# Nostrademous/dotaclient

Measured on AMD Instinct MI355X. Metric: PPO optimizer samples/sec (whole node) + actor steps/sec, 1v1-mid LSTM policy, higher is better.
Workload: dtype fp32

## Files before the change

dotaclient_amd/ops/csrc/dx_chain.hip:

```cpp
#include "common.h"
#include <cstdlib>

namespace {

using dca::bf16x8;
using dca::f32x4;

constexpr int BM = 48, BK = 32, NT = 512, P = 256, XC = 128, RD = 4;
constexpr int NI1 = BM / 16;

template <bool EXACT>
struct Lay {
  static constexpr int RP = EXACT ? 144 : 64;
  static constexpr int IMG = EXACT ? 1 : 2;
  static constexpr int A1 = BM * RP;
  static constexpr int B1 = P * RP;
  static constexpr int S1 = IMG * (A1 + B1);
  static constexpr int D = IMG * (P / BK) * A1;
  static constexpr int B2 = XC * RP;
  static constexpr int S2 = IMG * B2;
  static constexpr int BYTES = (2 * S1 > D + 2 * S2) ? 2 * S1 : D + 2 * S2;
};

template <bool EXACT>
__device__ __forceinline__ int coff(int r, int c) {
  if constexpr (EXACT) return r * Lay<true>::RP + 16 * c;
  else return r * 64 + 16 * (c ^ ((r >> 1) & 3));
}

__device__ __forceinline__ __amdgpu_buffer_rsrc_t rsrc(const void* p, long long bytes) {
  const unsigned long long a = (unsigned long long)p;
  const unsigned lo = __builtin_amdgcn_readfirstlane((unsigned)a);
  const unsigned hi = __builtin_amdgcn_readfirstlane((unsigned)(a >> 32));
  const int nb = (int)(bytes > 0x7fff0000LL ? 0x7fff0000LL : bytes);
  return __builtin_amdgcn_make_buffer_rsrc((void*)(((unsigned long long)hi << 32) | lo), (short)0,
                                           __builtin_amdgcn_readfirstlane(nb), 0x00020000);
}
__device__ __forceinline__ uint4 ld16(__amdgpu_buffer_rsrc_t r, int off) {
  return __builtin_bit_cast(uint4, __builtin_amdgcn_raw_buffer_load_b128(r, off, 0, 0));
}
constexpr int kOob = 0x7fff8000;

__device__ __forceinline__ unsigned pack2(short a, short b) {
  return (unsigned)(unsigned short)a | ((unsigned)(unsigned short)b << 16);
}
__device__ __forceinline__ void split4(const float4 v, uint2& hi, uint2& lo) {
  const short h0 = dca::f2bf(v.x), h1 = dca::f2bf(v.y), h2 = dca::f2bf(v.z), h3 = dca::f2bf(v.w);
  hi = make_uint2(pack2(h0, h1), pack2(h2, h3));
  lo = make_uint2(pack2(dca::f2bf(v.x - dca::bf2f(h0)), dca::f2bf(v.y - dca::bf2f(h1))),
                  pack2(dca::f2bf(v.z - dca::bf2f(h2)), dca::f2bf(v.w - dca::bf2f(h3))));
}

struct Frag {
  bf16x8 hi, lo;
  float f[8];
};
template <bool EXACT>
__device__ __forceinline__ void get_frag(const char* img, int img_bytes, int r, int q, Frag& fr) {
  if constexpr (EXACT) {
    const float4 a = *reinterpret_cast<const float4*>(img + coff<true>(r, 2 * q));
    const float4 b = *reinterpret_cast<const float4*>(img + coff<true>(r, 2 * q + 1));
    fr.f[0] = a.x; fr.f[1] = a.y; fr.f[2] = a.z; fr.f[3] = a.w;
    fr.f[4] = b.x; fr.f[5] = b.y; fr.f[6] = b.z; fr.f[7] = b.w;
  } else {
    const int o = coff<false>(r, q);
    fr.hi = *reinterpret_cast<const bf16x8*>(img + o);
    fr.lo = *reinterpret_cast<const bf16x8*>(img + img_bytes + o);
  }
}
template <bool EXACT, int NI, int NJ>
__device__ __forceinline__ void mma_tiles(const Frag (&fa)[NI], const Frag (&fb)[NJ], f32x4 (&acc)[NI][NJ]) {
  if constexpr (EXACT) {
#pragma unroll
    for (int e = 0; e < 8; ++e)
#pragma unroll
      for (int i = 0; i < NI; ++i)
#pragma unroll
        for (int j = 0; j < NJ; ++j)
          acc[i][j] = __builtin_amdgcn_mfma_f32_16x16x4f32(fa[i].f[e], fb[j].f[e], acc[i][j], 0, 0, 0);
  } else {
#pragma unroll
    for (int i = 0; i < NI; ++i)
#pragma unroll
      for (int j = 0; j < NJ; ++j) acc[i][j] = __builtin_amdgcn_mfma_f32_16x16x32_bf16(fa[i].lo, fb[j].hi, acc[i][j], 0, 0, 0);
#pragma unroll
    for (int i = 0; i < NI; ++i)
#pragma unroll
      for (int j = 0; j < NJ; ++j) acc[i][j] = __builtin_amdgcn_mfma_f32_16x16x32_bf16(fa[i].hi, fb[j].lo, acc[i][j], 0, 0, 0);
#pragma unroll
    for (int i = 0; i < NI; ++i)
#pragma unroll
      for (int j = 0; j < NJ; ++j) acc[i][j] = __builtin_amdgcn_mfma_f32_16x16x32_bf16(fa[i].hi, fb[j].hi, acc[i][j], 0, 0, 0);
  }
}

template <bool EXACT, int EPI>
__global__ __launch_bounds__(NT, 1) void dpre_dx_kernel(const float* __restrict__ dG, const void* __restrict__ w1h,
                                                        const void* __restrict__ w1l, const float* __restrict__ x,
                                                        const void* __restrict__ w2h, const void* __restrict__ w2l,
                                                        float* __restrict__ dpre, float* __restrict__ dx, int N,
                                                        int K1, int X) {
  using L = Lay<EXACT>;
  constexpr int ES = EXACT ? 4 : 2;
  __shared__ __attribute__((aligned(16))) char lds[L::BYTES];
  const int tid = threadIdx.x, w = tid >> 6, lane = tid & 63, r16 = lane & 15, q = lane >> 4;
  const int r0 = blockIdx.x * BM;
  const __amdgpu_buffer_rsrc_t rA = rsrc(dG, (long long)N * K1 * 4);
  const __amdgpu_buffer_rsrc_t rW1h = rsrc(w1h, (long long)P * K1 * ES);
  const __amdgpu_buffer_rsrc_t rW1l = rsrc(EXACT ? w1h : w1l, (long long)P * K1 * ES);
  const __amdgpu_buffer_rsrc_t rW2h = rsrc(w2h, (long long)X * P * ES);
  const __amdgpu_buffer_rsrc_t rW2l = rsrc(EXACT ? w2h : w2l, (long long)X * P * ES);

  char* dimg = lds;
  constexpr int DIMG = (P / BK) * L::A1;
  if (K1 > 0) {
  const int ar = tid >> 3, ak = (tid & 7) * 4;
  const int arow = r0 + ar;
  const int a_off0 = (ar < BM && arow < N) ? (arow * K1 + ak) * 4 : kOob;
  const int br = tid & 255, bh = tid >> 8;
  const int b_off0 = (br * K1 + 16 * bh) * ES;
  float4 sa[RD];
  uint4 sb[RD][4];
  auto load1 = [&](int slot, int k0) {
    const bool in = k0 < K1;
    sa[slot] = __builtin_bit_cast(float4, ld16(rA, (in && a_off0 != kOob) ? a_off0 + k0 * 4 : kOob));
    if constexpr (EXACT) {
#pragma unroll
      for (int i = 0; i < 4; ++i) sb[slot][i] = ld16(rW1h, in ? b_off0 + (k0 + 4 * i) * 4 : kOob);
    } else {
      const int o = (k0 / BK) * (P * 64) + tid * 16;
#pragma unroll
      for (int j = 0; j < 2; ++j) {
        sb[slot][j] = ld16(rW1h, in ? o + 8192 * j : kOob);
        sb[slot][2 + j] = ld16(rW1l, in ? o + 8192 * j : kOob);
      }
    }
  };
  auto store1 = [&](int slot, int buf) {
    char* base = lds + buf * L::S1;
    char* bb = base + L::IMG * L::A1;
    if constexpr (EXACT) {
      if (ar < BM) *reinterpret_cast<float4*>(base + ar * L::RP + ak * 4) = sa[slot];
#pragma unroll
      for (int i = 0; i < 4; ++i) *reinterpret_cast<uint4*>(bb + br * L::RP + (16 * bh + 4 * i) * 4) = sb[slot][i];
    } else {
      uint2 hi, lo;
      split4(sa[slot], hi, lo);
      const int o = coff<false>(ar, ak >> 3) + 8 * ((ak >> 2) & 1);
      if (ar < BM) {
        *reinterpret_cast<uint2*>(base + o) = hi;
        *reinterpret_cast<uint2*>(base + L::A1 + o) = lo;
      }
#pragma unroll
      for (int j = 0; j < 2; ++j) {
        const int ob = coff<false>(128 * j + (tid >> 2), tid & 3);
        *reinterpret_cast<uint4*>(bb + ob) = sb[slot][j];
        *reinterpret_cast<uint4*>(bb + L::B1 + ob) = sb[slot][2 + j];
      }
    }
  };
  const int wc = w;
  f32x4 acc[NI1][2];
#pragma unroll
  for (int i = 0; i < NI1; ++i)
#pragma unroll
    for (int j = 0; j < 2; ++j) acc[i][j] = f32x4{0.f, 0.f, 0.f, 0.f};
  const int nk = K1 / BK;
#pragma unroll
  for (int d = 0; d < RD; ++d) load1(d, d * BK);
  store1(0, 0);
  __syncthreads();
  for (int ks0 = 0; ks0 < nk; ks0 += RD) {
#pragma unroll
    for (int d = 0; d < RD; ++d) {
      const int ks = ks0 + d;
      const char* base = lds + (d & 1) * L::S1;
      const char* bb = base + L::IMG * L::A1;
      Frag fa[NI1], fb[2];
#pragma unroll
      for (int i = 0; i < NI1; ++i) get_frag<EXACT>(base, L::A1, i * 16 + r16, q, fa[i]);
#pragma unroll
      for (int j = 0; j < 2; ++j) get_frag<EXACT>(bb, L::B1, wc * 32 + j * 16 + r16, q, fb[j]);
      mma_tiles<EXACT, NI1, 2>(fa, fb, acc);
      store1((d + 1) % RD, (d + 1) & 1);
      load1(d, (ks + RD) * BK);
      __syncthreads();
    }
  }

  {
    const __amdgpu_buffer_rsrc_t rX = rsrc(x, EPI == 0 ? (long long)N * P * 4 : (long long)P * 4);
    float xv[NI1][2][4];
#pragma unroll
    for (int i = 0; i < NI1; ++i)
#pragma unroll
      for (int j = 0; j < 2; ++j)
#pragma unroll
        for (int e = 0; e < 4; ++e) {
          const int row = i * 16 + 4 * q + e, col = wc * 32 + j * 16 + r16;
          const int grow = r0 + row;
          if constexpr (EPI == 0) {
            xv[i][j][e] = __builtin_bit_cast(float, __builtin_amdgcn_raw_buffer_load_b32(
                              rX, grow < N ? (grow * P + col) * 4 : kOob, 0, 0));
          } else {
            xv[i][j][e] = e == 0 && i == 0 ? __builtin_bit_cast(float, __builtin_amdgcn_raw_buffer_load_b32(
                                                                           rX, col * 4, 0, 0))
                                           : 0.f;
          }
        }
    const __amdgpu_buffer_rsrc_t rD = rsrc(dpre, (long long)N * P * 4);
#pragma unroll
    for (int i = 0; i < NI1; ++i)
#pragma unroll
      for (int j = 0; j < 2; ++j)
#pragma unroll
        for (int e = 0; e < 4; ++e) {
          const int row = i * 16 + 4 * q + e, col = wc * 32 + j * 16 + r16;
          const int grow = r0 + row;
          float v;
          if constexpr (EPI == 0) v = xv[i][j][e] > 0.f ? acc[i][j][e] : 0.f;
          else if constexpr (EPI == 1) v = fmaxf(acc[i][j][e] + xv[0][j][0], 0.f);
          else v = acc[i][j][e] + xv[0][j][0];
          if (grow >= N) v = 0.f;
          __builtin_amdgcn_raw_buffer_store_b32(__builtin_bit_cast(unsigned, v), rD,
                                                grow < N ? (grow * P + col) * 4 : kOob, 0, 0);
          const int kk = col & (BK - 1);
          char* slab = dimg + (col / BK) * L::A1;
          if constexpr (EXACT) {
            *reinterpret_cast<float*>(slab + coff<true>(row, kk >> 2) + 4 * (kk & 3)) = v;
          } else {
            const int o = coff<false>(row, kk >> 3) + 2 * (kk & 7);
            const short h = dca::f2bf(v);
            *reinterpret_cast<short*>(slab + o) = h;
            *reinterpret_cast<short*>(slab + DIMG + o) = dca::f2bf(v - dca::bf2f(h));
          }
        }
  }

  } else if constexpr (EXACT) {
    for (int i = tid; i < BM * P / 4; i += NT) {
      const int row = i / (P / 4), c4 = (i % (P / 4)) * 4;
      const int grow = r0 + row;
      const float4 v = grow < N ? *reinterpret_cast<const float4*>(dG + (size_t)grow * P + c4)
                                : make_float4(0.f, 0.f, 0.f, 0.f);
      const int kk = c4 & (BK - 1);
      *reinterpret_cast<float4*>(dimg + (c4 / BK) * L::A1 + coff<true>(row, kk >> 2)) = v;
    }
  } else {
    for (int i = tid; i < BM * P / 4; i += NT) {
      const int row = i / (P / 4), c4 = (i % (P / 4)) * 4;
      const int grow = r0 + row;
      const float4 v = grow < N ? *reinterpret_cast<const float4*>(dG + (size_t)grow * P + c4)
                                : make_float4(0.f, 0.f, 0.f, 0.f);
      uint2 hi, lo;
      split4(v, hi, lo);
      const int kk = c4 & (BK - 1);
      char* slab = dimg + (c4 / BK) * L::A1;
      const int o = coff<false>(row, kk >> 3) + 2 * (kk & 7);
      *reinterpret_cast<uint2*>(slab + o) = hi;
      *reinterpret_cast<uint2*>(slab + DIMG + o) = lo;
    }
  }

  if (X == 0) return;
  char* s2 = lds + L::D;
  constexpr int nk2 = P / BK;
  const int nchunk = X / XC, total = nchunk * nk2;
  const int cr = tid & 127, cq = tid >> 7;
  uint4 sw[RD][2];
  auto load2 = [&](int slot, int it) {
    const int c0 = (it / nk2) * XC, kb = it % nk2;
    if constexpr (EXACT) {
      const int o = it < total ? ((c0 + cr) * P + kb * BK + 8 * cq) * ES : kOob;
      sw[slot][0] = ld16(rW2h, o);
      sw[slot][1] = ld16(rW2h, o + 16);
    } else {
      const int o = it < total ? (kb * X + c0) * 64 + tid * 16 : kOob;
      sw[slot][0] = ld16(rW2h, o);
      sw[slot][1] = ld16(rW2l, o);
    }
  };
  auto store2 = [&](int slot, int buf) {
    char* bb = s2 + buf * L::S2;
    if constexpr (EXACT) {
      *reinterpret_cast<uint4*>(bb + coff<true>(cr, 2 * cq)) = sw[slot][0];
      *reinterpret_cast<uint4*>(bb + coff<true>(cr, 2 * cq + 1)) = sw[slot][1];
    } else {
      const int o = coff<false>(tid >> 2, tid & 3);
      *reinterpret_cast<uint4*>(bb + o) = sw[slot][0];
      *reinterpret_cast<uint4*>(bb + L::B2 + o) = sw[slot][1];
    }
  };
  const int vc = w;
  f32x4 acc2[NI1][1];
#pragma unroll
  for (int i = 0; i < NI1; ++i) acc2[i][0] = f32x4{0.f, 0.f, 0.f, 0.f};
  const __amdgpu_buffer_rsrc_t rDx = rsrc(dx, (long long)N * X * 4);
#pragma unroll
  for (int d = 0; d < RD; ++d) load2(d, d);
  store2(0, 0);
  __syncthreads();
  for (int it0 = 0; it0 < total; it0 += RD) {
#pragma unroll
    for (int d = 0; d < RD; ++d) {
      const int it = it0 + d;
      const int chunk = it / nk2, ks = it % nk2;
      const char* bb = s2 + (d & 1) * L::S2;
      Frag fa[NI1], fb[1];
#pragma unroll
      for (int i = 0; i < NI1; ++i) get_frag<EXACT>(dimg + ks * L::A1, DIMG, i * 16 + r16, q, fa[i]);
      get_frag<EXACT>(bb, L::B2, vc * 16 + r16, q, fb[0]);
      mma_tiles<EXACT, NI1, 1>(fa, fb, acc2);
      store2((d + 1) % RD, (d + 1) & 1);
      load2(d, it + RD);
      if (ks == nk2 - 1) {
#pragma unroll
        for (int i = 0; i < NI1; ++i) {
#pragma unroll
          for (int e = 0; e < 4; ++e) {
            const int grow = r0 + i * 16 + 4 * q + e;
            const float v = acc2[i][0][e];
            __builtin_amdgcn_raw_buffer_store_b32(__builtin_bit_cast(unsigned, v), rDx,
                                                  grow < N ? (grow * X + chunk * XC + vc * 16 + r16) * 4 : kOob, 0, 0);
          }
          acc2[i][0] = f32x4{0.f, 0.f, 0.f, 0.f};
        }
      }
      __syncthreads();
    }
  }
}

__global__ __launch_bounds__(256) void split_bf16x2_kernel(const float4* __restrict__ src, uint2* __restrict__ hi,
                                                           uint2* __restrict__ lo, int n4) {
  const int i = blockIdx.x * 256 + threadIdx.x;
  if (i < n4) split4(src[i], hi[i], lo[i]);
}

__global__ __launch_bounds__(256) void split_bf16x2_blk_kernel(const float4* __restrict__ src, uint2* __restrict__ hi,
                                                               uint2* __restrict__ lo, int R, int K) {
  const int i = blockIdx.x * 256 + threadIdx.x;
  if (i >= R * (K / 4)) return;
  const int r = (4 * i) / K, k = (4 * i) % K;
  const int o4 = ((((k >> 5) * R + r) << 5) + (k & 31)) >> 2;
  split4(src[i], hi[o4], lo[o4]);
}

}

extern "C" hipError_t dca_split_bf16x2_blk(const float* src, short* hi, short* lo, int R, int K, hipStream_t stream) {
  if (K % 32 != 0 || R < 1) return hipErrorInvalidValue;
  const int n4 = R * (K / 4);
  hipLaunchKernelGGL(split_bf16x2_blk_kernel, dim3((n4 + 255) / 256), dim3(256), 0, stream,
                     reinterpret_cast<const float4*>(src), reinterpret_cast<uint2*>(hi), reinterpret_cast<uint2*>(lo),
                     R, K);
  return hipGetLastError();
}

extern "C" hipError_t dca_split_bf16x2(const float* src, short* hi, short* lo, long long n, hipStream_t stream) {
  if (n % 4 != 0) return hipErrorInvalidValue;
  const int n4 = (int)(n / 4);
  if (n4 == 0) return hipSuccess;
  hipLaunchKernelGGL(split_bf16x2_kernel, dim3((n4 + 255) / 256), dim3(256), 0, stream,
                     reinterpret_cast<const float4*>(src), reinterpret_cast<uint2*>(hi), reinterpret_cast<uint2*>(lo),
                     n4);
  return hipGetLastError();
}

extern "C" hipError_t dca_dpre_dx(const float* dG, const void* w1h, const void* w1l, const float* x, const void* w2h,
                                  const void* w2l, float* dpre, float* dx, int N, int K1, int X, int exact,
                                  int epi, hipStream_t stream) {
  if (N < 1 || (K1 == 0 && X == 0) || K1 < 0 || K1 % (RD * BK) != 0 || X < 0 || X % XC != 0 ||
      ((X / XC) * (P / BK)) % RD != 0 || epi < 0 || epi > 2)
    return hipErrorInvalidValue;
  if ((long long)N * K1 * 4 > 0x7fff0000LL) return hipErrorInvalidValue;
  const int grid = (N + BM - 1) / BM;
#define DCA_DX_LAUNCH(EX, EP)                                                                                    \
  hipLaunchKernelGGL((dpre_dx_kernel<EX, EP>), dim3(grid), dim3(NT), 0, stream, dG, w1h, w1l, x, w2h, w2l, dpre, dx, \
                     N, K1, X)
  if (exact) {
    if (epi == 0) DCA_DX_LAUNCH(true, 0);
    else if (epi == 1) DCA_DX_LAUNCH(true, 1);
    else DCA_DX_LAUNCH(true, 2);
  } else {
    if (epi == 0) DCA_DX_LAUNCH(false, 0);
    else if (epi == 1) DCA_DX_LAUNCH(false, 1);
    else DCA_DX_LAUNCH(false, 2);
  }
#undef DCA_DX_LAUNCH
  return hipGetLastError();
}
```

dotaclient_amd/ops/csrc/encoder.hip:

```cpp
#include "common.h"

namespace {

using dca::bf16x8;
using dca::bf16x4;
using dca::f32x4;

constexpr int kD = 128;
constexpr int kF = 10;
constexpr int kRows = 32;
constexpr int kLd = kD + 8;
constexpr int kJobs = 3;

struct Layout {
  int U;
  int cnt[6];
  int off[6];
};

struct FwdParams {
  const float* units;
  const float* env;
  const float* w1;
  const float* b1;
// ... 753 lines not shown
  if (job >= P.jbase[6]) return;
  const int cnt = P.L.cnt[tau], uoff = P.L.off[tau];
  const int NB = (N + 15) >> 4;
  const int g0 = (job - P.jbase[tau]) * P.gpj[tau], g1 = min(g0 + P.gpj[tau], NB);
  const int k0 = g0 * cnt, k1 = g1 * cnt, kl = k1 - 1;
  __shared__ __attribute__((aligned(16))) short img[2][2][kImg];
  __shared__ __attribute__((aligned(16))) float stg[3][kStg];

  const int col = 16 * wv + i;
  bf16x8 wf[4], wfl[4], wb;
#pragma unroll
  for (int s = 0; s < 4; ++s) {
    const float* p = P.wt + ((size_t)tau * kD + col) * kD + 32 * s + 8 * kg;
    const float4 a = *reinterpret_cast<const float4*>(p), b = *reinterpret_cast<const float4*>(p + 4);
    const float v[8] = {a.x, a.y, a.z, a.w, b.x, b.y, b.z, b.w};
#pragma unroll
    for (int jj = 0; jj < 8; ++jj) {
      wf[s][jj] = dca::f2bf(v[jj]);
      wfl[s][jj] = dca::f2bf(v[jj] - dca::bf2f(wf[s][jj]));
    }
  }
#pragma unroll
  for (int jj = 0; jj < 8; ++jj) {
    const int slot = 8 * kg + jj, f = l1_feat(slot);
    const float w = f >= 0 ? P.w1[col * kF + f] : P.b1[col];
    const short hi = dca::f2bf(w);
    const short lo = dca::f2bf(w - dca::bf2f(hi));
    wb[jj] = (slot == 31 || (f >= 0 && l1_wlo(slot))) ? lo : hi;
  }
  const float btv = P.bt[tau * kD + col];
  const __amdgpu_buffer_rsrc_t Ru = uniform_rsrc(P.units, N * U * kF * 4),
                               Re = uniform_rsrc(P.emb, N * U * kD * 4);
  f32x4 pmax = {-INFINITY, -INFINITY, -INFINITY, -INFINITY};
  int parg[4] = {0, 0, 0, 0};

  float pre = 0.f;
  if (wv < 3) {
    stg[k0 % 3][64 * wv + lane] = ff_stage_load(P, Ru, k0, cnt, uoff, wv, lane);
    stg[(k0 + 1) % 3][64 * wv + lane] = ff_stage_load(P, Ru, min(k0 + 1, kl), cnt, uoff, wv, lane);
    pre = ff_stage_load(P, Ru, min(k0 + 2, kl), cnt, uoff, wv, lane);
  }
  lds_barrier();
  ff_layer1(stg[k0 % 3], wb, &img[0][0][0], &img[0][1][0], wv, lane);
  int buf = 0;
  for (int k = k0; k < k1; ++k) {
    lds_barrier();
    if (wv < 3) {
      stg[(k + 2) % 3][64 * wv + lane] = pre;
      pre = ff_stage_load(P, Ru, min(k + 3, kl), cnt, uoff, wv, lane);
    }
    const int rb = k / cnt, u = k - rb * cnt, row0 = 16 * rb;
    const short* ih = &img[buf][0][0];
    const short* il = &img[buf][1][0];
    bf16x8 af[4], afl[4];
#pragma unroll
    for (int s = 0; s < 4; ++s) {
      af[s] = tile_frag(ih, 32 * s, lane);
      afl[s] = tile_frag(il, 32 * s, lane);
    }
    const f32x4 c = mfma3_k128(af, afl, wf, wfl);
    ff_layer1(stg[(k + 1) % 3], wb, &img[buf ^ 1][0][0], &img[buf ^ 1][1][0], wv, lane);
#pragma unroll
    for (int r = 0; r < 4; ++r) {
      const float v = c[r] + btv;
      if (v > pmax[r]) { pmax[r] = v; parg[r] = u; }
      const int row = row0 + 4 * kg + r;
      __builtin_amdgcn_raw_buffer_store_b32(__builtin_bit_cast(unsigned, v), Re, ((row * U + uoff + u) * kD + col) * 4,
                                            0, 0);
    }
    if (u == cnt - 1) {
#pragma unroll
      for (int r = 0; r < 4; ++r) {
        const int row = row0 + 4 * kg + r;
        if (row < N) {
          P.x896[(size_t)row * 896 + kD + tau * kD + col] = pmax[r];
          P.arg[((size_t)row * 6 + tau) * kD + col] = (unsigned char)parg[r];
        }
        pmax[r] = -INFINITY;
        parg[r] = 0;
      }
    }
    buf ^= 1;
  }
}

constexpr int kXP = 132;
constexpr int kXT = 20;

__device__ __forceinline__ f32x4 x_layer1(const float* sl, const float (&w1x)[3], int i, int kg) {
  f32x4 c = {0.f, 0.f, 0.f, 0.f};
#pragma unroll
  for (int cc = 0; cc < 3; ++cc) {
    const int f = 4 * cc + kg;
    const float a = f < kF ? sl[i * kF + f] : (f == kF ? 1.f : 0.f);
    c = __builtin_amdgcn_mfma_f32_16x16x4f32(a, w1x[cc], c, 0, 0, 0);
  }
  return c;
}

__device__ __forceinline__ void x_load_w1(const float* w1, const float* b1, int col, int kg, float (&w1x)[3]) {
#pragma unroll
  for (int cc = 0; cc < 3; ++cc) {
    const int f = 4 * cc + kg;
    w1x[cc] = f < kF ? w1[col * kF + f] : (f == kF ? b1[col] : 0.f);
  }
}

__device__ __forceinline__ void x_afrags(const float* img, int i, int kg, float (&a)[32]) {
#pragma unroll
  for (int s = 0; s < 4; ++s) {
    const float4 p = *reinterpret_cast<const float4*>(img + i * kXP + 32 * s + 8 * kg);
    const float4 q = *reinterpret_cast<const float4*>(img + i * kXP + 32 * s + 8 * kg + 4);
    a[8 * s + 0] = p.x; a[8 * s + 1] = p.y; a[8 * s + 2] = p.z; a[8 * s + 3] = p.w;
    a[8 * s + 4] = q.x; a[8 * s + 5] = q.y; a[8 * s + 6] = q.z; a[8 * s + 7] = q.w;
  }
}

__device__ __forceinline__ f32x4 x_mma_k128(const float (&a)[32], const float (&w)[32]) {
  f32x4 c0 = {0.f, 0.f, 0.f, 0.f}, c1 = {0.f, 0.f, 0.f, 0.f};
#pragma unroll
  for (int k = 0; k < 32; k += 2) {
    c0 = __builtin_amdgcn_mfma_f32_16x16x4f32(a[k], w[k], c0, 0, 0, 0);
    c1 = __builtin_amdgcn_mfma_f32_16x16x4f32(a[k + 1], w[k + 1], c1, 0, 0, 0);
  }
  return c0 + c1;
}

__device__ __forceinline__ void x_put(float* img, int n, const f32x4& v, int i, int kg) {
#pragma unroll
  for (int r = 0; r < 4; ++r) img[(4 * kg + r) * kXP + 16 * n + i] = v[r];
}

__global__ __launch_bounds__(512, 1) void encoder_fwd_x_kernel(FfParams P) {
  const int tid = threadIdx.x, wv = tid >> 6, lane = tid & 63;
  const int i = lane & 15, kg = lane >> 4;
  const int job = blockIdx.x, N = P.N, U = P.L.U;
  for (int rbase = 32 * job; rbase < N; rbase += 32 * (int)gridDim.x) {
    const int row = rbase + (tid >> 4), c0 = (tid & 15) * 8;
    if (row < N) {
      const float e0 = P.env[row * 3], e1 = P.env[row * 3 + 1], e2 = P.env[row * 3 + 2];
#pragma unroll
      for (int c = c0; c < c0 + 8; ++c)
        P.x896[(size_t)row * 896 + c] = fmaxf(P.be[c] + P.we[c * 3] * e0 + P.we[c * 3 + 1] * e1 + P.we[c * 3 + 2] * e2, 0.f);
    }
  }
  int tau = 0;
#pragma unroll
  for (int t = 1; t < 6; ++t) tau += job >= P.jbase[t] ? 1 : 0;
  if (job >= P.jbase[6]) return;
  const int cnt = P.L.cnt[tau], uoff = P.L.off[tau];
  const int NB = (N + 15) >> 4;
  const int g0 = (job - P.jbase[tau]) * P.gpj[tau], g1 = min(g0 + P.gpj[tau], NB);
  const int k0 = g0 * cnt, k1 = g1 * cnt, kl = k1 - 1;
  __shared__ __attribute__((aligned(16))) float img[2][16 * kXP];
  __shared__ __attribute__((aligned(16))) float stg[3][kStg];

  const int col = 16 * wv + i;
  float wx[32], w1x[3];
#pragma unroll
  for (int s = 0; s < 4; ++s) {
    const float* p = P.wt + ((size_t)tau * kD + col) * kD + 32 * s + 8 * kg;
    const float4 a = *reinterpret_cast<const float4*>(p), b = *reinterpret_cast<const float4*>(p + 4);
    wx[8 * s + 0] = a.x; wx[8 * s + 1] = a.y; wx[8 * s + 2] = a.z; wx[8 * s + 3] = a.w;
    wx[8 * s + 4] = b.x; wx[8 * s + 5] = b.y; wx[8 * s + 6] = b.z; wx[8 * s + 7] = b.w;
  }
  x_load_w1(P.w1, P.b1, col, kg, w1x);
  const float btv = P.bt[tau * kD + col];
  const __amdgpu_buffer_rsrc_t Ru = uniform_rsrc(P.units, N * U * kF * 4),
                               Re = uniform_rsrc(P.emb, N * U * kD * 4);
  f32x4 pmax = {-INFINITY, -INFINITY, -INFINITY, -INFINITY};
  int parg[4] = {0, 0, 0, 0};

  float pre = 0.f;
  if (wv < 3) {
    stg[k0 % 3][64 * wv + lane] = ff_stage_load(P, Ru, k0, cnt, uoff, wv, lane);
    stg[(k0 + 1) % 3][64 * wv + lane] = ff_stage_load(P, Ru, min(k0 + 1, kl), cnt, uoff, wv, lane);
    pre = ff_stage_load(P, Ru, min(k0 + 2, kl), cnt, uoff, wv, lane);
  }
  lds_barrier();
  {
    f32x4 b = x_layer1(stg[k0 % 3], w1x, i, kg);
#pragma unroll
    for (int r = 0; r < 4; ++r) b[r] = fmaxf(b[r], 0.f);
    x_put(img[0], wv, b, i, kg);
  }
  __builtin_amdgcn_s_waitcnt(0);
  int buf = 0;
  for (int k = k0; k < k1; ++k) {
    lds_barrier();
    const int rb = k / cnt, u = k - rb * cnt, row0 = 16 * rb;
    float a[32];
    x_afrags(img[buf], i, kg, a);
    const f32x4 c = x_mma_k128(a, wx);
    if (wv < 3) stg[(k + 2) % 3][64 * wv + lane] = pre;
    {
      f32x4 b = x_layer1(stg[(k + 1) % 3], w1x, i, kg);
#pragma unroll
      for (int r = 0; r < 4; ++r) b[r] = fmaxf(b[r], 0.f);
      x_put(img[buf ^ 1], wv, b, i, kg);
    }
#pragma unroll
    for (int r = 0; r < 4; ++r) {
      const float v = c[r] + btv;
      if (v > pmax[r]) { pmax[r] = v; parg[r] = u; }
      const int row = row0 + 4 * kg + r;
      __builtin_amdgcn_raw_buffer_store_b32(__builtin_bit_cast(unsigned, v), Re, ((row * U + uoff + u) * kD + col) * 4,
                                            0, 0);
    }
    if (u == cnt - 1) {
#pragma unroll
      for (int r = 0; r < 4; ++r) {
        const int row = row0 + 4 * kg + r;
        if (row < N) {
          P.x896[(size_t)row * 896 + kD + tau * kD + col] = pmax[r];
          P.arg[((size_t)row * 6 + tau) * kD + col] = (unsigned char)parg[r];
        }
        pmax[r] = -INFINITY;
        parg[r] = 0;
      }
    }
    if (wv < 3) pre = ff_stage_load(P, Ru, min(k + 3, kl), cnt, uoff, wv, lane);
    buf ^= 1;
  }
}

template <bool GIVEN>
__device__ __forceinline__ void xb_build(const FbBuild& b, const float* slot, int u, float* im, float* it, int wv,
                                         int lane) {
  const int i = lane & 15, kg = lane >> 4;
  f32x4 v;
  if constexpr (GIVEN) {
#pragma unroll
    for (int r = 0; r < 4; ++r) v[r] = b.q[r];
  } else {
    const f32x4 d4 = *reinterpret_cast<const f32x4*>(slot + 16 * kF + 4 * kg);
#pragma unroll
    for (int r = 0; r < 4; ++r) v[r] = d4[r] * b.q[r] + (b.ab[r] == (unsigned)u ? b.ds[r] : 0.f);
  }
  x_put(im, wv, v, i, kg);
  *reinterpret_cast<f32x4*>(it + (16 * wv + i) * kXT + 4 * kg) = v;
}

template <bool GIVEN, bool COMPAT>
__global__ __launch_bounds__(256, 2) void encoder_bwd_x2_kernel(FbParams P) {
  const int tid = threadIdx.x, w = tid >> 6, lane = tid & 63;
  const int i = lane & 15, kg = lane >> 4;
  const int job = blockIdx.x;
  int tau = 0;
#pragma unroll
  for (int t = 1; t < 6; ++t) tau += job >= P.jbase[t] ? 1 : 0;
  const int cnt = P.L.cnt[tau], uoff = P.L.off[tau], N = P.N, U = P.L.U;
  const int NB = (N + 15) >> 4;
  const int k0 = (job - P.jbase[tau]) * P.items, k1 = min(k0 + P.items, cnt * NB);
  __shared__ __attribute__((aligned(16))) float img[2][16 * kXP];
  __shared__ __attribute__((aligned(16))) float imt[2][128 * kXT];
  __shared__ __attribute__((aligned(16))) float stg[3][kStg];
  FbRsrc R;
  if constexpr (GIVEN) {
    R.g = uniform_rsrc(P.demb_in, N * U * kD * 4);
  } else {
    R.q = uniform_rsrc(P.q, N * P.ldq * 4);
    R.x = uniform_rsrc(P.dx, N * 896 * 4);
    R.a = uniform_rsrc(P.arg, N * 6 * kD);
  }

  float wx[2][32], w1x[2][3];
#pragma unroll
  for (int t = 0; t < 2; ++t) {
    const int col = 16 * (2 * w + t) + i;
#pragma unroll
    for (int s = 0; s < 4; ++s) {
      const float* p = P.wtT + ((size_t)tau * kD + col) * kD + 32 * s + 8 * kg;
      const float4 a = *reinterpret_cast<const float4*>(p), b = *reinterpret_cast<const float4*>(p + 4);
      wx[t][8 * s + 0] = a.x; wx[t][8 * s + 1] = a.y; wx[t][8 * s + 2] = a.z; wx[t][8 * s + 3] = a.w;
      wx[t][8 * s + 4] = b.x; wx[t][8 * s + 5] = b.y; wx[t][8 * s + 6] = b.z; wx[t][8 * s + 7] = b.w;
    }
    x_load_w1(P.w1, P.b1, col, kg, w1x[t]);
  }
  f32x4 acc[2][8], dw1acc[2] = {{0.f, 0.f, 0.f, 0.f}, {0.f, 0.f, 0.f, 0.f}};
  float db1acc[2] = {0.f, 0.f};
#pragma unroll
  for (int t = 0; t < 2; ++t)
#pragma unroll
    for (int et = 0; et < 8; ++et) acc[t][et] = f32x4{0.f, 0.f, 0.f, 0.f};

  FbBuild bn[2];
  const int kl = max(k1 - 1, 0);
  float pre = 0.f;
  if (w < 3) {
    stg[k0 % 3][64 * w + lane] = fb_stage_load(P, min(k0, kl), cnt, uoff, w, lane);
    stg[(k0 + 1) % 3][64 * w + lane] = fb_stage_load(P, min(k0 + 1, kl), cnt, uoff, w, lane);
    pre = fb_stage_load(P, min(k0 + 2, kl), cnt, uoff, w, lane);
  }
#pragma unroll
  for (int t = 0; t < 2; ++t)
    fb_load_build<GIVEN, COMPAT>(bn[t], R, P.ldq, min(k0, kl), true, cnt, uoff, U, tau, 2 * w + t, i, kg);
  lds_barrier();
#pragma unroll
  for (int t = 0; t < 2; ++t) xb_build<GIVEN>(bn[t], stg[k0 % 3], k0 % cnt, img[0], imt[0], 2 * w + t, lane);
#pragma unroll
  for (int t = 0; t < 2; ++t)
    fb_load_build<GIVEN, COMPAT>(bn[t], R, P.ldq, min(k0 + 1, kl), min(k0 + 1, kl) % cnt == 0, cnt, uoff, U, tau,
                                 2 * w + t, i, kg);
  float l1n[3], ubn[4];
  auto l1_read = [&](const float* sl) {
#pragma unroll
    for (int cc = 0; cc < 3; ++cc) {
      const int f = 4 * cc + kg;
      l1n[cc] = f < kF ? sl[i * kF + f] : (f == kF ? 1.f : 0.f);
    }
#pragma unroll
    for (int r = 0; r < 4; ++r) ubn[r] = i < kF ? sl[(4 * kg + r) * kF + i] : 0.f;
  };
  l1_read(stg[k0 % 3]);
  int buf = 0;
  for (int k = k0; k < k1; ++k) {
    lds_barrier();
    float a[32];
    x_afrags(img[buf], i, kg, a);
    const float ub[4] = {ubn[0], ubn[1], ubn[2], ubn[3]};
    f32x4 bas[2], c[2];
#pragma unroll
    for (int t = 0; t < 2; ++t) {
      bas[t] = f32x4{0.f, 0.f, 0.f, 0.f};
#pragma unroll
      for (int cc = 0; cc < 3; ++cc) bas[t] = __builtin_amdgcn_mfma_f32_16x16x4f32(l1n[cc], w1x[t][cc], bas[t], 0, 0, 0);
    }
    {
      f32x4 c0 = {0.f, 0.f, 0.f, 0.f}, c1 = c0, d0 = c0, d1 = c0;
#pragma unroll
      for (int kk = 0; kk < 32; kk += 2) {
        c0 = __builtin_amdgcn_mfma_f32_16x16x4f32(a[kk], wx[0][kk], c0, 0, 0, 0);
        d0 = __builtin_amdgcn_mfma_f32_16x16x4f32(a[kk], wx[1][kk], d0, 0, 0, 0);
      }
#pragma unroll
      for (int kk = 1; kk < 32; kk += 2) {
        c1 = __builtin_amdgcn_mfma_f32_16x16x4f32(a[kk], wx[0][kk], c1, 0, 0, 0);
        d1 = __builtin_amdgcn_mfma_f32_16x16x4f32(a[kk], wx[1][kk], d1, 0, 0, 0);
      }
      c[0] = c0 + c1;
      c[1] = d0 + d1;
    }
    f32x4 et4[8];
#pragma unroll
    for (int et = 0; et < 8; ++et) et4[et] = *reinterpret_cast<const f32x4*>(imt[buf] + (16 * et + i) * kXT + 4 * kg);
    if (w < 3) stg[(k + 2) % 3][64 * w + lane] = pre;
#pragma unroll
    for (int t = 0; t < 2; ++t)
      xb_build<GIVEN>(bn[t], stg[(k + 1) % 3], min(k + 1, kl) % cnt, img[buf ^ 1], imt[buf ^ 1], 2 * w + t, lane);
#pragma unroll
    for (int t = 0; t < 2; ++t)
      fb_load_build<GIVEN, COMPAT>(bn[t], R, P.ldq, min(k + 2, kl), k + 2 <= kl && (k + 2) % cnt == 0, cnt, uoff, U,
                                   tau, 2 * w + t, i, kg);
    l1_read(stg[(k + 1) % 3]);
    if (w < 3) pre = fb_stage_load(P, min(k + 3, kl), cnt, uoff, w, lane);
#pragma unroll
    for (int t = 0; t < 2; ++t)
#pragma unroll
      for (int r = 0; r < 4; ++r) bas[t][r] = fmaxf(bas[t][r], 0.f);
#pragma unroll
    for (int et = 0; et < 8; ++et) {
      f32x4 p0 = __builtin_amdgcn_mfma_f32_16x16x4f32(bas[0][0], et4[et][0], f32x4{0.f, 0.f, 0.f, 0.f}, 0, 0, 0);
      f32x4 p1 = __builtin_amdgcn_mfma_f32_16x16x4f32(bas[1][0], et4[et][0], f32x4{0.f, 0.f, 0.f, 0.f}, 0, 0, 0);
#pragma unroll
      for (int r = 1; r < 4; ++r) {
        p0 = __builtin_amdgcn_mfma_f32_16x16x4f32(bas[0][r], et4[et][r], p0, 0, 0, 0);
        p1 = __builtin_amdgcn_mfma_f32_16x16x4f32(bas[1][r], et4[et][r], p1, 0, 0, 0);
      }
      acc[0][et] += p0;
      acc[1][et] += p1;
    }
#pragma unroll
    for (int t = 0; t < 2; ++t) {
#pragma unroll
      for (int r = 0; r < 4; ++r) {
        c[t][r] = bas[t][r] > 0.f ? c[t][r] : 0.f;
        db1acc[t] += c[t][r];
      }
      f32x4 p1 = {0.f, 0.f, 0.f, 0.f};
#pragma unroll
      for (int r = 0; r < 4; ++r) p1 = __builtin_amdgcn_mfma_f32_16x16x4f32(c[t][r], ub[r], p1, 0, 0, 0);
      dw1acc[t] += p1;
    }
    buf ^= 1;
  }
  float* dst = P.dwtpart + (size_t)job * (kD * kD);
  float* wp = P.w1part + (size_t)job * kW1;
#pragma unroll
  for (int t = 0; t < 2; ++t) {
    const int jt = 2 * w + t;
#pragma unroll
    for (int et = 0; et < 8; ++et) *reinterpret_cast<f32x4*>(dst + ((8 * jt + et) * 64 + lane) * 4) = acc[t][et];
    if (i < kF) {
#pragma unroll
      for (int r = 0; r < 4; ++r) wp[(16 * jt + 4 * kg + r) * kF + i] = dw1acc[t][r];
    }
    float s = db1acc[t];
    s += __shfl_xor(s, 16, 64);
    s += __shfl_xor(s, 32, 64);
    if (kg == 0) wp[kD * kF + 16 * jt + i] = s;
  }
}

__global__ __launch_bounds__(256) void fb_dwt_reduce(const float* __restrict__ part, FbParams P, float* __restrict__ dwt) {
  __shared__ float red[4][64];
  const int tau = blockIdx.y, ph = threadIdx.x >> 6;
  const int xi = blockIdx.x * 64 + (threadIdx.x & 63);
  float s = 0.f;
#pragma unroll 4
  for (int j = P.jbase[tau] + ph; j < P.jbase[tau + 1]; j += 4) s += part[(size_t)j * (kD * kD) + xi];
  red[ph][threadIdx.x & 63] = s;
  __syncthreads();
  if (ph) return;
  s = ((red[0][threadIdx.x] + red[1][threadIdx.x]) + red[2][threadIdx.x]) + red[3][threadIdx.x];
  const int r = xi & 3, lane = (xi >> 2) & 63, tile = xi >> 8;
  const int j = 16 * (tile >> 3) + 4 * (lane >> 4) + r;
  const int e = 16 * (tile & 7) + (lane & 15);
  dwt[(size_t)tau * kD * kD + e * kD + j] = s;
}

__global__ __launch_bounds__(256) void encoder_w1_reduce(const float* __restrict__ part, int nblk,
                                                          float* __restrict__ dw1, float* __restrict__ db1) {
  __shared__ float red[16][16];
  const int c = blockIdx.x * 16 + (threadIdx.x & 15), ph = threadIdx.x >> 4;
  float s = 0.f;
  if (c < kW1) {
#pragma unroll 4
    for (int b = ph; b < nblk; b += 16) s += part[(size_t)b * kW1 + c];
  }
  red[ph][threadIdx.x & 15] = s;
  __syncthreads();
  if (ph == 0 && c < kW1) {
    float v = 0.f;
#pragma unroll
    for (int k = 0; k < 16; ++k) v += red[k][threadIdx.x];
    if (c < kD * kF) dw1[c] = v;
    else db1[c - kD * kF] = v;
  }
}


constexpr int kJobBlk = 64;
struct DwtJobs {
  long long blkbase[6];
  int nblk[6];
  int jbase[7];
};

__device__ __forceinline__ void dwt_load(const short* __restrict__ A, const short* __restrict__ Bm, long long b,
                                         long long bend, int mq, int nq, int lane, bf16x8 (&a)[4], bf16x8 (&bb)[4]) {
  const long long blk = b + (lane >> 5);
  const bool ok = blk < bend;
  const int kh = 8 * ((lane >> 4) & 1);
#pragma unroll
  for (int t = 0; t < 4; ++t) {
    const size_t oa = ((size_t)blk * kD + 64 * mq + 16 * t + (lane & 15)) * 16 + kh;
    const size_t ob = ((size_t)blk * kD + 64 * nq + 16 * t + (lane & 15)) * 16 + kh;
    a[t] = ok ? *reinterpret_cast<const bf16x8*>(A + oa) : bf16x8{};
    bb[t] = ok ? *reinterpret_cast<const bf16x8*>(Bm + ob) : bf16x8{};
  }
}

__global__ __launch_bounds__(256, 2) void dwt_blocked_kernel(const short* __restrict__ A, const short* __restrict__ Bm,
                                                             DwtJobs J, float* __restrict__ part) {
  const int job = blockIdx.x, wv = threadIdx.x >> 6, lane = threadIdx.x & 63;
  int tau = 0;
  while (tau < 5 && job >= J.jbase[tau + 1]) ++tau;
  const long long b0 = J.blkbase[tau] + (long long)(job - J.jbase[tau]) * kJobBlk;
  const long long bend = min(b0 + kJobBlk, J.blkbase[tau] + J.nblk[tau]);
  const int mq = wv >> 1, nq = wv & 1;
  f32x4 acc[4][4];
#pragma unroll
  for (int x = 0; x < 4; ++x)
#pragma unroll
    for (int y = 0; y < 4; ++y) acc[x][y] = f32x4{0.f, 0.f, 0.f, 0.f};
  bf16x8 a[4], bb[4], an[4], bn[4];
  dwt_load(A, Bm, b0, bend, mq, nq, lane, a, bb);
  for (long long b = b0; b < bend; b += 2) {
    if (b + 2 < bend) dwt_load(A, Bm, b + 2, bend, mq, nq, lane, an, bn);
#pragma unroll
    for (int x = 0; x < 4; ++x)
#pragma unroll
      for (int y = 0; y < 4; ++y) acc[x][y] = __builtin_amdgcn_mfma_f32_16x16x32_bf16(a[x], bb[y], acc[x][y], 0, 0, 0);
#pragma unroll
    for (int t = 0; t < 4; ++t) {
      a[t] = an[t];
      bb[t] = bn[t];
    }
  }
  float* dst = part + (size_t)job * (kD * kD) + (size_t)wv * 16 * 256;
#pragma unroll
  for (int x = 0; x < 4; ++x)
#pragma unroll
    for (int y = 0; y < 4; ++y) *reinterpret_cast<f32x4*>(dst + ((4 * x + y) * 64 + lane) * 4) = acc[x][y];
}

__global__ __launch_bounds__(256) void dwt_reduce(const float* __restrict__ part, DwtJobs J, float* __restrict__ dwt) {
  __shared__ float red[4][64];
  const int tau = blockIdx.y, ph = threadIdx.x >> 6;
  const int xi = blockIdx.x * 64 + (threadIdx.x & 63);
  float s = 0.f;
#pragma unroll 4
  for (int j = J.jbase[tau] + ph; j < J.jbase[tau + 1]; j += 4) s += part[(size_t)j * (kD * kD) + xi];
  red[ph][threadIdx.x & 63] = s;
  __syncthreads();
  if (ph) return;
  s = ((red[0][threadIdx.x] + red[1][threadIdx.x]) + red[2][threadIdx.x]) + red[3][threadIdx.x];
  const int r = xi & 3, lane = (xi >> 2) & 63, tile = (xi >> 8) & 15, wv = xi >> 12;
  const int m = 64 * (wv >> 1) + 16 * (tile >> 2) + 4 * (lane >> 4) + r;
  const int n = 64 * (wv & 1) + 16 * (tile & 3) + (lane & 15);
  dwt[(size_t)tau * kD * kD + m * kD + n] = s;
}

}

extern "C" hipError_t dca_encoder_fwd(const float* units, const float* env, const float* w1, const float* b1,
                                      const void* wt, const float* bt, const float* we, const float* be, void* x896,
                                      void* emb, unsigned char* arg, int N, int U, const int* counts, int compat,
                                      hipStream_t st, int f32) {
  FwdParams P{units, env, w1, b1, wt, bt, we, be, x896, emb, arg, N, compat, {}};
  P.L.U = U;
  int acc = 0;
  for (int t = 0; t < 6; ++t) { P.L.cnt[t] = counts[t]; P.L.off[t] = acc; acc += counts[t]; }
  if (acc != U || U > 64) return hipErrorInvalidValue;
  if (f32) {
    FfParams F{units, env, w1, b1, static_cast<const float*>(wt), bt, we, be, static_cast<float*>(x896),
               static_cast<float*>(emb), arg, N, P.L, {}, {}};
    const long long NB = (N + 15) / 16;
    long long total = 0;
    for (int t = 0; t < 6; ++t) total += counts[t] * NB;
    const long long target = std::max<long long>(1, (total + 499) / 500);
    int jobs = 0;
    for (int t = 0; t < 6; ++t) {
      F.jbase[t] = jobs;
      F.gpj[t] = (int)((target + std::max(1, counts[t]) - 1) / std::max(1, counts[t]));
      if (counts[t] > 0) jobs += (int)((NB + F.gpj[t] - 1) / F.gpj[t]);
    }
    F.jbase[6] = jobs;
    if (f32 == 2) encoder_fwd_x_kernel<<<std::max(jobs, 1), 512, 0, st>>>(F);
    else encoder_fwd_f32_items_kernel<<<std::max(jobs, 1), 512, 0, st>>>(F);
    return hipGetLastError();
  }
  const dim3 grid((N + kRows - 1) / kRows, kJobs);
  encoder_fwd_kernel<<<grid, 256, 0, st>>>(P);
  return hipGetLastError();
}

namespace {
void dwt_plan(int N, const int* counts, DwtJobs& J, int& NB) {
  NB = (N + 15) / 16;
  long long acc = 0;
  int jobs = 0;
  for (int t = 0; t < 6; ++t) {
    J.blkbase[t] = acc;
    J.nblk[t] = counts[t] * NB;
    J.jbase[t] = jobs;
    acc += J.nblk[t];
    jobs += (J.nblk[t] + kJobBlk - 1) / kJobBlk;
  }
  J.jbase[6] = jobs;
}

void fb_plan(int N, const int* counts, FbParams& P) {
  const long long NB = (N + 15) / 16;
  long long total = 0;
  for (int t = 0; t < 6; ++t) total += counts[t] * NB;
  P.items = (int)std::max<long long>(1, (total + 499) / 500);
  int jobs = 0;
  for (int t = 0; t < 6; ++t) {
    P.jbase[t] = jobs;
    jobs += (int)((counts[t] * NB + P.items - 1) / P.items);
  }
  P.jbase[6] = jobs;
}
}

extern "C" size_t dca_encoder_bwd_workspace(int N, int U, const int* counts, int f32) {
  if (f32) {
    FbParams F{};
    fb_plan(N, counts, F);
    return (size_t)F.jbase[6] * (kW1 + kD * kD) * sizeof(float);
  }
  DwtJobs J;
  int NB;
  dwt_plan(N, counts, J, NB);
  const size_t w1 = (size_t)((N + kRows - 1) / kRows) * kJobs * kW1 * sizeof(float);
  const size_t img = (size_t)U * NB * kD * 16 * sizeof(short);
  const size_t parts = (size_t)J.jbase[6] * kD * kD * sizeof(float);
  return w1 + 2 * img + parts;
}

extern "C" hipError_t dca_encoder_bwd(const float* units, const float* w1, const float* b1, const void* wtT,
                                      const float* dtl, const float* q, int ldq, const float* dx,
                                      const unsigned char* arg, float* dwt, float* dw1, float* db1, void* ws,
                                      size_t ws_bytes, int N, int U, const int* counts, int compat, hipStream_t st,
                                      const void* demb_in, int f32) {
  if (ws_bytes < dca_encoder_bwd_workspace(N, U, counts, f32)) return hipErrorInvalidValue;
  int acc = 0;
  for (int t = 0; t < 6; ++t) acc += counts[t];
  if (acc != U || U > 64) return hipErrorInvalidValue;
  if (f32) {
    FbParams F{units, w1, b1, static_cast<const float*>(wtT), dtl, q, ldq, dx, arg,
               static_cast<const float*>(demb_in), nullptr, nullptr, N, compat, 0, {}, {}};
    fb_plan(N, counts, F);
    F.L.U = U;
    for (int t = 0, o = 0; t < 6; ++t) { F.L.cnt[t] = counts[t]; F.L.off[t] = o; o += counts[t]; }
    const int jobs = F.jbase[6];
    F.w1part = static_cast<float*>(ws);
    F.dwtpart = F.w1part + (size_t)jobs * kW1;
    if (jobs > 0 && f32 == 2) {
      if (demb_in) encoder_bwd_x2_kernel<true, false><<<jobs, 256, 0, st>>>(F);
      else if (compat) encoder_bwd_x2_kernel<false, true><<<jobs, 256, 0, st>>>(F);
      else encoder_bwd_x2_kernel<false, false><<<jobs, 256, 0, st>>>(F);
    } else if (jobs > 0) {
      if (demb_in) encoder_bwd_f32_fused_kernel<true, false><<<jobs, 512, 0, st>>>(F);
      else if (compat) encoder_bwd_f32_fused_kernel<false, true><<<jobs, 512, 0, st>>>(F);
      else encoder_bwd_f32_fused_kernel<false, false><<<jobs, 512, 0, st>>>(F);
    }
    encoder_w1_reduce<<<(kW1 + 15) / 16, 256, 0, st>>>(F.w1part, jobs, dw1, db1);
    fb_dwt_reduce<<<dim3(kD * kD / 64, 6), 256, 0, st>>>(F.dwtpart, F, dwt);
    return hipGetLastError();
  }
  DwtJobs J;
  int NB;
  dwt_plan(N, counts, J, NB);
  const int nblk = (N + kRows - 1) / kRows;
  char* p = static_cast<char*>(ws);
  float* w1part = reinterpret_cast<float*>(p);
  p += (size_t)nblk * kJobs * kW1 * sizeof(float);
  const size_t img = (size_t)U * NB * kD * 16;
  short* demb = reinterpret_cast<short*>(p);
  short* basic = demb + img;
  float* parts = reinterpret_cast<float*>(basic + img);
  BwdParams P{units, w1, b1, wtT, dtl, q, ldq, dx, arg, demb, basic, w1part, N, compat, {}, {}, NB, demb_in};
  P.L.U = U;
  acc = 0;
  for (int t = 0; t < 6; ++t) {
    P.L.cnt[t] = counts[t];
    P.L.off[t] = acc;
    P.blkbase[t] = J.blkbase[t];
    acc += counts[t];
  }
  encoder_bwd_kernel<<<dim3(nblk, kJobs), 256, 0, st>>>(P);
  encoder_w1_reduce<<<(kW1 + 15) / 16, 256, 0, st>>>(w1part, nblk * kJobs, dw1, db1);
  if (J.jbase[6] > 0) dwt_blocked_kernel<<<J.jbase[6], 256, 0, st>>>(demb, basic, J, parts);
  dwt_reduce<<<dim3(kD * kD / 64, 6), 256, 0, st>>>(parts, J, dwt);
  return hipGetLastError();
}
```

Before: 1.989 million.

## Triple-buffer exact fp32 dx_chain GEMMs with split MFMA scheduling and coalesced loads

```diff
diff --git a/dotaclient_amd/ops/csrc/dx_chain.hip b/dotaclient_amd/ops/csrc/dx_chain.hip
--- a/dotaclient_amd/ops/csrc/dx_chain.hip
+++ b/dotaclient_amd/ops/csrc/dx_chain.hip
@@ -19,7 +19,9 @@
   static constexpr int D = IMG * (P / BK) * A1;
   static constexpr int B2 = XC * RP;
   static constexpr int S2 = IMG * B2;
-  static constexpr int BYTES = (2 * S1 > D + 2 * S2) ? 2 * S1 : D + 2 * S2;
+  static constexpr int NB = EXACT ? 3 : 2;
+  static constexpr int MAIN = (NB * S1 > D + NB * S2) ? NB * S1 : D + NB * S2;
+  static constexpr int BYTES = MAIN + (EXACT ? NT * 16 : 0);
 };
 
 template <bool EXACT>
@@ -68,11 +70,11 @@
     fr.lo = *reinterpret_cast<const bf16x8*>(img + img_bytes + o);
   }
 }
-template <bool EXACT, int NI, int NJ>
+template <bool EXACT, int NI, int NJ, int E0 = 0, int E1 = 8>
 __device__ __forceinline__ void mma_tiles(const Frag (&fa)[NI], const Frag (&fb)[NJ], f32x4 (&acc)[NI][NJ]) {
   if constexpr (EXACT) {
 #pragma unroll
-    for (int e = 0; e < 8; ++e)
+    for (int e = E0; e < E1; ++e)
 #pragma unroll
       for (int i = 0; i < NI; ++i)
 #pragma unroll
@@ -117,8 +119,8 @@
   const int ar = tid >> 3, ak = (tid & 7) * 4;
   const int arow = r0 + ar;
   const int a_off0 = (ar < BM && arow < N) ? (arow * K1 + ak) * 4 : kOob;
-  const int br = tid & 255, bh = tid >> 8;
-  const int b_off0 = (br * K1 + 16 * bh) * ES;
+  const int br = tid >> 3, bp = tid & 7;
+  const int b_off0 = (br * K1 + 4 * bp) * ES;
   float4 sa[RD];
   uint4 sb[RD][4];
   auto load1 = [&](int slot, int k0) {
@@ -126,7 +128,7 @@
     sa[slot] = __builtin_bit_cast(float4, ld16(rA, (in && a_off0 != kOob) ? a_off0 + k0 * 4 : kOob));
     if constexpr (EXACT) {
 #pragma unroll
-      for (int i = 0; i < 4; ++i) sb[slot][i] = ld16(rW1h, in ? b_off0 + (k0 + 4 * i) * 4 : kOob);
+      for (int i = 0; i < 4; ++i) sb[slot][i] = ld16(rW1h, in ? b_off0 + (64 * i * K1 + k0) * 4 : kOob);
     } else {
       const int o = (k0 / BK) * (P * 64) + tid * 16;
 #pragma unroll
@@ -136,13 +138,13 @@
       }
     }
   };
-  auto store1 = [&](int slot, int buf) {
-    char* base = lds + buf * L::S1;
+  auto store1 = [&](int slot, int boff) {
+    char* base = lds + boff;
     char* bb = base + L::IMG * L::A1;
     if constexpr (EXACT) {
-      if (ar < BM) *reinterpret_cast<float4*>(base + ar * L::RP + ak * 4) = sa[slot];
-#pragma unroll
-      for (int i = 0; i < 4; ++i) *reinterpret_cast<uint4*>(bb + br * L::RP + (16 * bh + 4 * i) * 4) = sb[slot][i];
+      *reinterpret_cast<float4*>(lds + (ar < BM ? boff + ar * L::RP + ak * 4 : L::MAIN + tid * 16)) = sa[slot];
+#pragma unroll
+      for (int i = 0; i < 4; ++i) *reinterpret_cast<uint4*>(bb + (br + 64 * i) * L::RP + 16 * bp) = sb[slot][i];
     } else {
       uint2 hi, lo;
       split4(sa[slot], hi, lo);
@@ -168,6 +170,44 @@
   const int nk = K1 / BK;
 #pragma unroll
   for (int d = 0; d < RD; ++d) load1(d, d * BK);
+  if constexpr (EXACT) {
+    int o0 = 0, o1 = L::S1, o2 = 2 * L::S1;
+    store1(0, o0);
+    store1(1, o1);
+    __syncthreads();
+    Frag fa[2][NI1], fb[2][2];
+    auto frags1 = [&](int set, int boff) {
+      const char* base = lds + boff;
+      const char* bb = base + L::A1;
+#pragma unroll
+      for (int i = 0; i < NI1; ++i) get_frag<true>(base, L::A1, i * 16 + r16, q, fa[set][i]);
+#pragma unroll
+      for (int j = 0; j < 2; ++j) get_frag<true>(bb, L::B1, wc * 32 + j * 16 + r16, q, fb[set][j]);
+    };
+    frags1(0, o0);
+    for (int ks0 = 0; ks0 < nk; ks0 += RD) {
+#pragma unroll
+      for (int d = 0; d < RD; ++d) {
+        const int ks = ks0 + d;
+        frags1((d + 1) & 1, o1);
+        mma_tiles<true, NI1, 2, 0, 4>(fa[d & 1], fb[d & 1], acc);
+        store1((d + 2) % RD, o2);
+        load1(d, (ks + RD) * BK);
+        mma_tiles<true, NI1, 2, 4, 8>(fa[d & 1], fb[d & 1], acc);
+        __builtin_amdgcn_sched_group_barrier(0x100, 10, 0);
+#pragma unroll
+        for (int g = 0; g < 5; ++g) {
+          __builtin_amdgcn_sched_group_barrier(0x008, 8, 0);
+          __builtin_amdgcn_sched_group_barrier(0x200, 1, 0);
+        }
+        __builtin_amdgcn_sched_group_barrier(0x008, 4, 0);
+        __builtin_amdgcn_sched_group_barrier(0x020, 5, 0);
+        __builtin_amdgcn_sched_group_barrier(0x008, 4, 0);
+        __syncthreads();
+        const int t = o0; o0 = o1; o1 = o2; o2 = t;
+      }
+    }
+  } else {
   store1(0, 0);
   __syncthreads();
   for (int ks0 = 0; ks0 < nk; ks0 += RD) {
@@ -182,10 +222,11 @@
 #pragma unroll
       for (int j = 0; j < 2; ++j) get_frag<EXACT>(bb, L::B1, wc * 32 + j * 16 + r16, q, fb[j]);
       mma_tiles<EXACT, NI1, 2>(fa, fb, acc);
-      store1((d + 1) % RD, (d + 1) & 1);
+      store1((d + 1) % RD, ((d + 1) & 1) * L::S1);
       load1(d, (ks + RD) * BK);
       __syncthreads();
     }
+  }
   }
 
   {
@@ -266,25 +307,25 @@
   char* s2 = lds + L::D;
   constexpr int nk2 = P / BK;
   const int nchunk = X / XC, total = nchunk * nk2;
-  const int cr = tid & 127, cq = tid >> 7;
+  const int cr = tid >> 3, cq = tid & 7;
   uint4 sw[RD][2];
   auto load2 = [&](int slot, int it) {
     const int c0 = (it / nk2) * XC, kb = it % nk2;
     if constexpr (EXACT) {
-      const int o = it < total ? ((c0 + cr) * P + kb * BK + 8 * cq) * ES : kOob;
+      const int o = it < total ? ((c0 + cr) * P + kb * BK + 4 * cq) * ES : kOob;
       sw[slot][0] = ld16(rW2h, o);
-      sw[slot][1] = ld16(rW2h, o + 16);
+      sw[slot][1] = ld16(rW2h, it < total ? o + 64 * P * ES : kOob);
     } else {
       const int o = it < total ? (kb * X + c0) * 64 + tid * 16 : kOob;
       sw[slot][0] = ld16(rW2h, o);
       sw[slot][1] = ld16(rW2l, o);
     }
   };
-  auto store2 = [&](int slot, int buf) {
-    char* bb = s2 + buf * L::S2;
+  auto store2 = [&](int slot, int boff) {
+    char* bb = s2 + boff;
     if constexpr (EXACT) {
-      *reinterpret_cast<uint4*>(bb + coff<true>(cr, 2 * cq)) = sw[slot][0];
-      *reinterpret_cast<uint4*>(bb + coff<true>(cr, 2 * cq + 1)) = sw[slot][1];
+      *reinterpret_cast<uint4*>(bb + coff<true>(cr, cq)) = sw[slot][0];
+      *reinterpret_cast<uint4*>(bb + coff<true>(cr + 64, cq)) = sw[slot][1];
     } else {
       const int o = coff<false>(tid >> 2, tid & 3);
       *reinterpret_cast<uint4*>(bb + o) = sw[slot][0];
@@ -298,6 +339,56 @@
   const __amdgpu_buffer_rsrc_t rDx = rsrc(dx, (long long)N * X * 4);
 #pragma unroll
   for (int d = 0; d < RD; ++d) load2(d, d);
+  auto out2 = [&](int chunk) {
+#pragma unroll
+    for (int i = 0; i < NI1; ++i) {
+#pragma unroll
+      for (int e = 0; e < 4; ++e) {
+        const int grow = r0 + i * 16 + 4 * q + e;
+        const float v = acc2[i][0][e];
+        __builtin_amdgcn_raw_buffer_store_b32(__builtin_bit_cast(unsigned, v), rDx,
+                                              grow < N ? (grow * X + chunk * XC + vc * 16 + r16) * 4 : kOob, 0, 0);
+      }
+      acc2[i][0] = f32x4{0.f, 0.f, 0.f, 0.f};
+    }
+  };
+  if constexpr (EXACT) {
+    int o0 = 0, o1 = L::S2, o2 = 2 * L::S2;
+    store2(0, o0);
+    store2(1, o1);
+    __syncthreads();
+    Frag fa[2][NI1], fb[2][1];
+    auto frags2 = [&](int set, int ks, int boff) {
+#pragma unroll
+      for (int i = 0; i < NI1; ++i) get_frag<true>(dimg + ks * L::A1, DIMG, i * 16 + r16, q, fa[set][i]);
+      get_frag<true>(s2 + boff, L::B2, vc * 16 + r16, q, fb[set][0]);
+    };
+    frags2(0, 0, o0);
+    for (int it0 = 0; it0 < total; it0 += RD) {
+#pragma unroll
+      for (int d = 0; d < RD; ++d) {
+        const int it = it0 + d;
+        const int chunk = it / nk2, ks = it % nk2;
+        frags2((d + 1) & 1, (ks + 1) % nk2, o1);
+        mma_tiles<true, NI1, 1, 0, 4>(fa[d & 1], fb[d & 1], acc2);
+        store2((d + 2) % RD, o2);
+        load2(d, it + RD);
+        mma_tiles<true, NI1, 1, 4, 8>(fa[d & 1], fb[d & 1], acc2);
+        __builtin_amdgcn_sched_group_barrier(0x100, 8, 0);
+#pragma unroll
+        for (int g = 0; g < 2; ++g) {
+          __builtin_amdgcn_sched_group_barrier(0x008, 8, 0);
+          __builtin_amdgcn_sched_group_barrier(0x200, 1, 0);
+        }
+        __builtin_amdgcn_sched_group_barrier(0x008, 4, 0);
+        __builtin_amdgcn_sched_group_barrier(0x020, 2, 0);
+        __builtin_amdgcn_sched_group_barrier(0x008, 4, 0);
+        if (ks == nk2 - 1) out2(chunk);
+        __syncthreads();
+        const int t = o0; o0 = o1; o1 = o2; o2 = t;
+      }
+    }
+  } else {
   store2(0, 0);
   __syncthreads();
   for (int it0 = 0; it0 < total; it0 += RD) {
@@ -311,23 +402,12 @@
       for (int i = 0; i < NI1; ++i) get_frag<EXACT>(dimg + ks * L::A1, DIMG, i * 16 + r16, q, fa[i]);
       get_frag<EXACT>(bb, L::B2, vc * 16 + r16, q, fb[0]);
       mma_tiles<EXACT, NI1, 1>(fa, fb, acc2);
-      store2((d + 1) % RD, (d + 1) & 1);
+      store2((d + 1) % RD, ((d + 1) & 1) * L::S2);
       load2(d, it + RD);
-      if (ks == nk2 - 1) {
-#pragma unroll
-        for (int i = 0; i < NI1; ++i) {
-#pragma unroll
-          for (int e = 0; e < 4; ++e) {
-            const int grow = r0 + i * 16 + 4 * q + e;
-            const float v = acc2[i][0][e];
-            __builtin_amdgcn_raw_buffer_store_b32(__builtin_bit_cast(unsigned, v), rDx,
-                                                  grow < N ? (grow * X + chunk * XC + vc * 16 + r16) * 4 : kOob, 0, 0);
-          }
-          acc2[i][0] = f32x4{0.f, 0.f, 0.f, 0.f};
-        }
-      }
+      if (ks == nk2 - 1) out2(chunk);
       __syncthreads();
     }
+  }
   }
 }
 
diff --git a/dotaclient_amd/ops/csrc/encoder.hip b/dotaclient_amd/ops/csrc/encoder.hip
--- a/dotaclient_amd/ops/csrc/encoder.hip
+++ b/dotaclient_amd/ops/csrc/encoder.hip
@@ -1079,30 +1079,21 @@
   for (int t = 0; t < 2; ++t)
     fb_load_build<GIVEN, COMPAT>(bn[t], R, P.ldq, min(k0 + 1, kl), min(k0 + 1, kl) % cnt == 0, cnt, uoff, U, tau,
                                  2 * w + t, i, kg);
-  float l1n[3], ubn[4];
-  auto l1_read = [&](const float* sl) {
-#pragma unroll
-    for (int cc = 0; cc < 3; ++cc) {
-      const int f = 4 * cc + kg;
-      l1n[cc] = f < kF ? sl[i * kF + f] : (f == kF ? 1.f : 0.f);
-    }
-#pragma unroll
-    for (int r = 0; r < 4; ++r) ubn[r] = i < kF ? sl[(4 * kg + r) * kF + i] : 0.f;
-  };
-  l1_read(stg[k0 % 3]);
   int buf = 0;
   for (int k = k0; k < k1; ++k) {
     lds_barrier();
     float a[32];
     x_afrags(img[buf], i, kg, a);
-    const float ub[4] = {ubn[0], ubn[1], ubn[2], ubn[3]};
+    const float* sl = stg[k % 3];
+    float l1n[3], ub[4];
+#pragma unroll
+    for (int cc = 0; cc < 3; ++cc) {
+      const int f = 4 * cc + kg;
+      l1n[cc] = f < kF ? sl[i * kF + f] : (f == kF ? 1.f : 0.f);
+    }
+#pragma unroll
+    for (int r = 0; r < 4; ++r) ub[r] = i < kF ? sl[(4 * kg + r) * kF + i] : 0.f;
     f32x4 bas[2], c[2];
-#pragma unroll
-    for (int t = 0; t < 2; ++t) {
-      bas[t] = f32x4{0.f, 0.f, 0.f, 0.f};
-#pragma unroll
-      for (int cc = 0; cc < 3; ++cc) bas[t] = __builtin_amdgcn_mfma_f32_16x16x4f32(l1n[cc], w1x[t][cc], bas[t], 0, 0, 0);
-    }
     {
       f32x4 c0 = {0.f, 0.f, 0.f, 0.f}, c1 = c0, d0 = c0, d1 = c0;
 #pragma unroll
@@ -1118,9 +1109,25 @@
       c[0] = c0 + c1;
       c[1] = d0 + d1;
     }
-    f32x4 et4[8];
-#pragma unroll
-    for (int et = 0; et < 8; ++et) et4[et] = *reinterpret_cast<const f32x4*>(imt[buf] + (16 * et + i) * kXT + 4 * kg);
+#pragma unroll
+    for (int t = 0; t < 2; ++t) {
+      bas[t] = f32x4{0.f, 0.f, 0.f, 0.f};
+#pragma unroll
+      for (int cc = 0; cc < 3; ++cc) bas[t] = __builtin_amdgcn_mfma_f32_16x16x4f32(l1n[cc], w1x[t][cc], bas[t], 0, 0, 0);
+    }
+#pragma unroll
+    for (int t = 0; t < 2; ++t) {
+#pragma unroll
+      for (int r = 0; r < 4; ++r) {
+        bas[t][r] = fmaxf(bas[t][r], 0.f);
+        c[t][r] = bas[t][r] > 0.f ? c[t][r] : 0.f;
+        db1acc[t] += c[t][r];
+      }
+      f32x4 p1 = {0.f, 0.f, 0.f, 0.f};
+#pragma unroll
+      for (int r = 0; r < 4; ++r) p1 = __builtin_amdgcn_mfma_f32_16x16x4f32(c[t][r], ub[r], p1, 0, 0, 0);
+      dw1acc[t] += p1;
+    }
     if (w < 3) stg[(k + 2) % 3][64 * w + lane] = pre;
 #pragma unroll
     for (int t = 0; t < 2; ++t)
@@ -1129,12 +1136,10 @@
     for (int t = 0; t < 2; ++t)
       fb_load_build<GIVEN, COMPAT>(bn[t], R, P.ldq, min(k + 2, kl), k + 2 <= kl && (k + 2) % cnt == 0, cnt, uoff, U,
                                    tau, 2 * w + t, i, kg);
-    l1_read(stg[(k + 1) % 3]);
     if (w < 3) pre = fb_stage_load(P, min(k + 3, kl), cnt, uoff, w, lane);
-#pragma unroll
-    for (int t = 0; t < 2; ++t)
-#pragma unroll
-      for (int r = 0; r < 4; ++r) bas[t][r] = fmaxf(bas[t][r], 0.f);
+    f32x4 et4[8];
+#pragma unroll
+    for (int et = 0; et < 8; ++et) et4[et] = *reinterpret_cast<const f32x4*>(imt[buf] + (16 * et + i) * kXT + 4 * kg);
 #pragma unroll
     for (int et = 0; et < 8; ++et) {
       f32x4 p0 = __builtin_amdgcn_mfma_f32_16x16x4f32(bas[0][0], et4[et][0], f32x4{0.f, 0.f, 0.f, 0.f}, 0, 0, 0);
@@ -1146,18 +1151,6 @@
       }
       acc[0][et] += p0;
       acc[1][et] += p1;
-    }
-#pragma unroll
-    for (int t = 0; t < 2; ++t) {
-#pragma unroll
-      for (int r = 0; r < 4; ++r) {
-        c[t][r] = bas[t][r] > 0.f ? c[t][r] : 0.f;
-        db1acc[t] += c[t][r];
-      }
-      f32x4 p1 = {0.f, 0.f, 0.f, 0.f};
-#pragma unroll
-      for (int r = 0; r < 4; ++r) p1 = __builtin_amdgcn_mfma_f32_16x16x4f32(c[t][r], ub[r], p1, 0, 0, 0);
-      dw1acc[t] += p1;
     }
     buf ^= 1;
   }
```

Result: faster. 2.015 million (median of 6 runs) (+1.3%).
